# fpthink/PDGN

Measured on AMD Instinct MI355X. Metric: generator+D step points/sec (B=35, 256->2048 pts), higher is better.
Workload: dtype f32; 1 GPU; PDGNet_v2 G+D iteration (models/PDGNet_v2.py:171-256), chair-shaped synthetic batch, per-GPU batch 35, 256->2048 pts, random-init weights; global_batch=35, parallelism=dp1, losses_finite=True, hipgraph=False, issue=list

## Files before the change

include/pdgn_hip.h:

```cpp
#ifndef PDGN_HIP_H
#define PDGN_HIP_H

#include <stdint.h>

#ifdef __cplusplus
extern "C" {
#endif

#define PDGN_ERR_INVALID (-1)
#define PDGN_KNN_MAX_NSAMPLE 200

typedef void *pdgn_stream_t;

int pdgn_abi_version(void);

int pdgn_knnquery(int b, int n, int m, int nsample, const float *xyz, const float *new_xyz,
                  int32_t *idx, float *dist2, pdgn_stream_t stream);

int pdgn_grouping_forward(int b, int c, int n, int m, int nsample, const float *points,
                          const int32_t *idx, float *out, pdgn_stream_t stream);

int pdgn_grouping_backward(int b, int c, int n, int m, int nsample, const float *grad_out,
                           const int32_t *idx, float *grad_points, pdgn_stream_t stream);

// ... 54 lines not shown
                  const float *beta, const float *pre_bias, float *running_mean, float *running_var,
                  float *scratch, float *stats, pdgn_stream_t stream);
int pdgn_bn_eval_stats(int c, float eps, const float *gamma, const float *beta, const float *pre_bias,
                       const float *running_mean, const float *running_var, float *stats,
                       pdgn_stream_t stream);
int pdgn_bn_stats_from_partials(long long rows, int c, float eps, float momentum, const float *gamma,
                                const float *beta, const float *pre_bias, float *running_mean, float *running_var,
                                const float *scratch, float *stats, pdgn_stream_t stream);
int pdgn_bn_stats_from_gemm_partials(long long rows, int c, long long nparts, int block_rows, float eps, float momentum,
                                     const float *gamma, const float *beta, const float *pre_bias,
                                     float *running_mean, float *running_var, const float *partials,
                                     float *stats, double *scratch, pdgn_stream_t stream);
long long pdgn_bn_blocks_scratch_doubles(int c, long long nparts);
int pdgn_bn_act_forward(long long rows, int c, int act, const float *x, const float *stats,
                        const float *mul, float *y, int interleave_n, pdgn_stream_t stream);
int pdgn_bn_act_backward(long long rows, int c, int act, int training, const float *x,
                         const float *dy, const float *mul, const float *stats, float *scratch,
                         float *bsums, float *dx, float *dmul, int interleave_n, pdgn_stream_t stream);

long long pdgn_bn_maxpool_scratch_floats(int b, int c);
int pdgn_bn_act_maxpool(int b, int n, int c, int act, const float *x, const float *stats, float *scratch,
                        float *ymax, int32_t *yarg, pdgn_stream_t stream);
long long pdgn_bn_stats_maxpool_scratch_floats(int b, int c);
int pdgn_bn_stats_act_maxpool(int b, int n, int c, int act, float eps, float momentum, const float *x, const float *gamma,
                              const float *beta, const float *pre_bias, float *running_mean, float *running_var, float *scratch,
                              float *stats, float *ymax, int32_t *yarg, pdgn_stream_t stream);
int pdgn_bn_act_maxpool_backward(int b, int n, int c, int act, int training, const float *x,
                                 const float *dout, const int32_t *yarg, const float *stats,
                                 float *scratch, float *bsums, float *dx, pdgn_stream_t stream);
long long pdgn_dense_bn_maxpool_backward_scratch(int b, int c, int k);
int pdgn_dense_bn_maxpool_backward(int b, int n, int c, int k, int act, const float *x, const float *dout, const int32_t *yarg,
                                   const float *stats, const float *h, int ldh, const float *W, int ldw, float *scratch,
                                   float *dh, float *dW, int lddw, float *bsums, pdgn_stream_t stream);
long long pdgn_dense_bn_maxpool_input_grad_scratch(int b, int c, int k);
int pdgn_dense_bn_maxpool_input_grad(int b, int n, int c, int k, int act, const float *x, const float *dout,
                                     const int32_t *yarg, const float *stats, const float *h, int ldh,
                                     const float *W, int ldw, float *scratch, float *dh, pdgn_stream_t stream);

int pdgn_group_colsum(long long groups, long long group_rows, int c, const float *x, long long ldx, float *out,
                      pdgn_stream_t stream);

int pdgn_softmax_slots_permute(long long m, int k, int c, const float *h, float *w, pdgn_stream_t stream);
int pdgn_bn_softmax_slots_permute(long long m, int k, int c, int act, const float *x, const float *stats,
                                  float *w, pdgn_stream_t stream);
int pdgn_bn_softmax_slots_permute_mul(long long m, int k, int c, int act, const float *x, const float *stats,
                                      int act_u, const float *u, const float *stats_u, float *w, float *y,
                                      unsigned *max_out, const float *gamma_u, const float *beta_u, float bound_scale,
                                      unsigned *cmax_out, pdgn_stream_t stream);
long long pdgn_bilateral_scratch_floats(long long m, int k, int c);
int pdgn_bilateral_weighting_backward(long long m, int k, int c, int act, int training, const float *x,
                                      const float *stats_x, const float *u, const float *stats_u, const float *w,
                                      const float *dy, float *scratch, float *bsums_x, float *bsums_u, float *dx,
                                      float *du, pdgn_stream_t stream);
int pdgn_softmax_slots_permute_backward(long long m, int k, int c, const float *w, const float *dw,
                                        float *dh, pdgn_stream_t stream);

int pdgn_skinny_nt(int R, int N, int K, const float *A, int lda, const float *B, int ldb, const float *bias, float *C, int ldc,
                   pdgn_stream_t stream);
int pdgn_skinny_nn(int R, int N, int K, const float *A, int lda, const float *B, int ldb, float *C, int ldc, pdgn_stream_t stream);
int pdgn_skinny_nt_act(int R, int N, int K, const float *A, int lda, const float *B, int ldb, const float *bias, float *C, int ldc,
                       int act, pdgn_stream_t stream);
int pdgn_skinny_nn_masked(int R, int N, int K, const float *A, int lda, const float *P, int ldp, int act, const float *B,
                          int ldb, float *C, int ldc, pdgn_stream_t stream);
int pdgn_skinny_tn(int R, int N, int K, const float *A, int lda, const float *B, int ldb, float *C, int ldc, pdgn_stream_t stream);
int pdgn_split_bf16x3(int rows, int cols, const float *src, int ld_src, unsigned short *planes, int ld_planes,
                      long long plane_stride, unsigned short *planes_t, int ld_planes_t, long long plane_stride_t,
// ... 149 lines not shown
```

pdgn_amd/_lib.py:

```python
import ctypes
import os

import torch

_HERE = os.path.dirname(os.path.abspath(__file__))
SO_PATH = os.path.join(_HERE, "libpdgn_hip.so")
ABI_VERSION = 26
_lib = None


class PdgnHipError(RuntimeError):
    pass


def lib():
    global _lib
    if _lib is None:
        if not os.path.exists(SO_PATH):
            raise PdgnHipError(
                "libpdgn_hip.so is not built (%s missing): run `python -m pdgn_amd.build`; "
                "pdgn_amd has no CPU fallback" % SO_PATH)
        handle = ctypes.CDLL(SO_PATH)
        handle.pdgn_abi_version.restype = ctypes.c_int
        got = handle.pdgn_abi_version()
        if got != ABI_VERSION:
            raise PdgnHipError("libpdgn_hip.so ABI %d != expected %d: rebuild" % (got, ABI_VERSION))
        _lib = handle
        if handle.pdgn_gemm_set_mode(-1) == 2:
            ensure_scale_slots(handle=handle)
    return _lib


_SCALE_SLOTS = {}


def ensure_scale_slots(device=None, handle=None):
    if not torch.cuda.is_available():
        return
    idx = torch.cuda.current_device() if device is None or device.index is None else device.index
    if _SCALE_SLOTS.get("attached") == idx:
# ... 66 lines not shown
```

pdgn_amd/csrc/bnact.hip:

```cpp
#include "common.h"

#include "bn_geom.h"
#define ACT_NONE 0
#define ACT_RELU 1
#define ACT_LEAKY 2

__device__ __forceinline__ float act_fwd(float z, int act) {
    if (act == ACT_RELU) return fmaxf(z, 0.f);
    if (act == ACT_LEAKY) return z > 0.f ? z : 0.01f * z;
    return z;
}
__device__ __forceinline__ float act_grad(float z, int act) {
    if (act == ACT_RELU) return z > 0.f ? 1.f : 0.f;
    if (act == ACT_LEAKY) return z > 0.f ? 1.f : 0.01f;
    return 1.f;
}

struct ClGeom {
    int cg, cgb, rl;
};

__global__ __launch_bounds__(BN_THREADS) void cl_stats_kernel(long long R, int C, int cgb, int rows_per_block,
                                                              const float *__restrict__ x,
                                                              float *__restrict__ part) {
// ... 900 lines not shown
        }
    }
    const size_t blk = (size_t)b * MP_SPLIT + sp;
    float *P = part + blk * 2 * C;
    *reinterpret_cast<float4 *>(P + cgi * 4) = make_float4(s[0], s[1], s[2], s[3]);
    *reinterpret_cast<float4 *>(P + C + cgi * 4) = make_float4(q[0], q[1], q[2], q[3]);
    const size_t o = blk * C + cgi * 4;
    *reinterpret_cast<float4 *>(pmax + o) = make_float4(mx[0], mx[1], mx[2], mx[3]);
    *reinterpret_cast<int4 *>(pargmax + o) = make_int4(amx[0], amx[1], amx[2], amx[3]);
    *reinterpret_cast<float4 *>(pmin + o) = make_float4(mn[0], mn[1], mn[2], mn[3]);
    *reinterpret_cast<int4 *>(pargmin + o) = make_int4(amn[0], amn[1], amn[2], amn[3]);
}

__global__ void cl_max_pick_kernel(int B, int C, int act, const float *__restrict__ stats, const float *__restrict__ pmax,
                                   const int32_t *__restrict__ pargmax, const float *__restrict__ pmin,
                                   const int32_t *__restrict__ pargmin, float *__restrict__ ymax, int32_t *__restrict__ yarg) {
    const int e = blockIdx.x * blockDim.x + threadIdx.x;
    if (e >= B * C) return;
    const int b = e / C, c = e - b * C;
    const float sc = stats[c], sh = stats[C + c];
    const bool up = sc >= 0.f;
    const float *pv = up ? pmax : pmin;
    const int32_t *pa = up ? pargmax : pargmin;
    float best = pv[((size_t)b * MP_SPLIT) * C + c];
    int arg = pa[((size_t)b * MP_SPLIT) * C + c];
    for (int s = 1; s < MP_SPLIT; ++s) {
        const float v = pv[((size_t)b * MP_SPLIT + s) * C + c];
        if (up ? v > best : v < best) { best = v; arg = pa[((size_t)b * MP_SPLIT + s) * C + c]; }
    }
    ymax[e] = act_fwd(__fmaf_rn(best, sc, sh), act);
    yarg[e] = arg;
}

__global__ __launch_bounds__(256) void cl_max_bwd_sums_kernel(int B, int N, int C, int act, int training,
                                                              const float *__restrict__ x, const float *__restrict__ dout,
                                                              const int32_t *__restrict__ yarg, const float *__restrict__ stats,
                                                              float *__restrict__ dz, float *__restrict__ bsums,
                                                              float *__restrict__ coef, float *__restrict__ zero, int nzero) {
    __shared__ double p1[16][17], p2[16][17];
    for (int e = blockIdx.x * 256 + threadIdx.x; e < nzero; e += gridDim.x * 256) zero[e] = 0.f;
    const int cl = threadIdx.x & 15, bl = threadIdx.x >> 4;
    const int c = blockIdx.x * 16 + cl;
    double s1 = 0, s2 = 0;
    float sc = 0.f, mu = 0.f, is = 0.f;
    if (c < C) {
        sc = stats[c];
        mu = stats[2 * C + c];
        is = stats[3 * C + c];
        const float sh = stats[C + c];
        for (int b = bl; b < B; b += 16) {
            const int n = yarg[b * C + c];
            const float v = x[((size_t)b * N + n) * C + c];
            const float g = dout[b * C + c] * act_grad(__fmaf_rn(v, sc, sh), act);
            dz[b * C + c] = g;
            s1 += g;
            s2 += (double)g * (double)((v - mu) * is);
        }
    }
    p1[bl][cl] = s1;
    p2[bl][cl] = s2;
    __syncthreads();
    if (bl || c >= C) return;
    for (int q = 1; q < 16; ++q) { s1 += p1[q][cl]; s2 += p2[q][cl]; }
    bsums[c] = (float)s1;
    bsums[C + c] = (float)s2;
    float ca = 0.f, cb = 0.f;
    if (training) {
        const double R = (double)B * (double)N;
        cb = sc * is * (float)(s2 / R);
        ca = sc * (float)(s1 / R) - cb * mu;
    }
    coef[c] = ca;
    coef[C + c] = cb;
}

__global__ __launch_bounds__(BN_THREADS) void cl_max_bwd_apply_kernel(int N, int C, int cgb, const float *__restrict__ x,
                                                                      const float *__restrict__ stats,
                                                                      const float *__restrict__ coef,
                                                                      const float *__restrict__ dz,
                                                                      const int32_t *__restrict__ yarg,
                                                                      float *__restrict__ dx) {
    const int cgl = threadIdx.x % cgb, rlane = threadIdx.x / cgb, rl = BN_THREADS / cgb;
    const int cgi = blockIdx.x * cgb + cgl;
    if (cgi * 4 >= C) return;
    const int b = blockIdx.z, sp = blockIdx.y;
// ... 37 lines not shown
    hipLaunchKernelGGL(cl_apply_max_kernel, dim3(gx, MP_SPLIT, b), dim3(BN_THREADS), 0, s, n, c, cgb, act, x, stats, pmax, parg);
    hipLaunchKernelGGL(cl_max_finalize_kernel, dim3(cdiv((long long)b * c, 256)), dim3(256), 0, s, b, c, pmax, parg, ymax, yarg);
    return pdgn_launch_status();
}

extern "C" long long pdgn_bn_stats_maxpool_scratch_floats(int b, int c) { return 6LL * b * MP_SPLIT * c; }

extern "C" int pdgn_bn_stats_act_maxpool(int b, int n, int c, int act, float eps, float momentum, const float *x, const float *gamma,
                                         const float *beta, const float *pre_bias, float *running_mean, float *running_var,
                                         float *scratch, float *stats, float *ymax, int32_t *yarg, pdgn_stream_t stream) {
    if (b < 1 || n < 1 || c < 4 || c % 4 || act < 0 || act > 2 || b > 65535) return PDGN_ERR_INVALID;
    hipStream_t s = (hipStream_t)stream;
    int cgb, gx;
    mp_geometry(c, &cgb, &gx);
    const size_t bc = (size_t)b * MP_SPLIT * c;
    float *part = scratch, *pmax = part + 2 * bc, *pmin = pmax + 2 * bc;
    int32_t *pargmax = reinterpret_cast<int32_t *>(pmax + bc), *pargmin = reinterpret_cast<int32_t *>(pmin + bc);
    hipLaunchKernelGGL(cl_stats_max_kernel, dim3(gx, MP_SPLIT, b), dim3(BN_THREADS), 0, s, n, c, cgb, x, part, pmax, pargmax, pmin,
                       pargmin);
    hipLaunchKernelGGL(cl_finalize_kernel, dim3(cdiv(c, FIN_CH)), dim3(FIN_CH * FIN_PL), 0, s, (long long)b * n, c, b * MP_SPLIT, eps,
                       momentum, part, gamma, beta, pre_bias, running_mean, running_var, stats, x);
    hipLaunchKernelGGL(cl_max_pick_kernel, dim3(cdiv((long long)b * c, 256)), dim3(256), 0, s, b, c, act, stats, pmax, pargmax, pmin,
                       pargmin, ymax, yarg);
    return pdgn_launch_status();
}

extern "C" int pdgn_bn_act_maxpool_backward(int b, int n, int c, int act, int training, const float *x,
                                            const float *dout, const int32_t *yarg, const float *stats, float *scratch,
                                            float *bsums, float *dx, pdgn_stream_t stream) {
    if (b < 1 || n < 1 || c < 4 || c % 4 || act < 0 || act > 2 || b > 65535) return PDGN_ERR_INVALID;
    hipStream_t s = (hipStream_t)stream;
    float *dz = scratch, *coef = scratch + (size_t)b * c;
    hipLaunchKernelGGL(cl_max_bwd_sums_kernel, dim3(cdiv(c, 16)), dim3(256), 0, s, b, n, c, act, training, x, dout, yarg,
                       stats, dz, bsums, coef, nullptr, 0);
    int cgb, gx;
    mp_geometry(c, &cgb, &gx);
    hipLaunchKernelGGL(cl_max_bwd_apply_kernel, dim3(gx, MP_SPLIT, b), dim3(BN_THREADS), 0, s, n, c, cgb, x, stats, coef, dz,
                       yarg, dx);
    return pdgn_launch_status();
}

#define CF_TILE 32
#define CF_CSPLIT 8
#define CF_RSPLIT 32

__global__ __launch_bounds__(256) void cf_gram_kernel(int C, int K, const float *__restrict__ W, int ldw,
                                                      const float *__restrict__ coef, float *__restrict__ Gneg,
                                                      float *__restrict__ vneg) {
    __shared__ float part[3][64][20];
    const int t = threadIdx.x, o = t & 63, sl = __builtin_amdgcn_readfirstlane(t >> 6);
    const int i = blockIdx.y * CF_TILE + (o >> 3) * 4, j = blockIdx.x * CF_TILE + (o & 7) * 4;
    const bool ok = i < K && j < K, do_v = blockIdx.y == 0 && (o >> 3) == 0 && j < K;
    const int ii = min(i, K - 4), jj = min(j, K - 4);
    const int nsl = CF_CSPLIT * 4, per = (C + nsl - 1) / nsl;
    const int c0 = (blockIdx.z * 4 + sl) * per, c1 = min(C, c0 + per);
    const float *cb = coef + C;
    float acc[4][4] = {}, av[4] = {};
    for (int c = c0; c < c1; c += 8) {
        float4 wi[8], wj[8];
#pragma unroll
        for (int u = 0; u < 8; ++u) {
            const float *w = W + (size_t)min(c + u, c1 - 1) * ldw;
            wi[u] = *reinterpret_cast<const float4 *>(w + ii);
            wj[u] = *reinterpret_cast<const float4 *>(w + jj);
        }
        __builtin_amdgcn_sched_barrier(0);
#pragma unroll
// ... 152 lines not shown
                                                    float *__restrict__ dW, int lddw) {
    const int lane = threadIdx.x & 63, c = blockIdx.x * 4 + (threadIdx.x >> 6);
    if (c >= C || lane * 4 >= K) return;
    const int col = lane * 4;
    const float sc = stats[c];
    float4 acc = make_float4(0.f, 0.f, 0.f, 0.f);
    for (int b0 = 0; b0 < B; b0 += 8) {
        float4 v[8];
        float g[8];
#pragma unroll
        for (int u = 0; u < 8; ++u) {
            const int b = min(b0 + u, B - 1);
            g[u] = b0 + u < B ? sc * dz[(size_t)b * C + c] : 0.f;
            v[u] = *reinterpret_cast<const float4 *>(h + ((size_t)b * N + yarg[(size_t)b * C + c]) * ldh + col);
        }
#pragma unroll
        for (int u = 0; u < 8; ++u) {
            acc.x = __fmaf_rn(g[u], v[u].x, acc.x);
            acc.y = __fmaf_rn(g[u], v[u].y, acc.y);
            acc.z = __fmaf_rn(g[u], v[u].z, acc.z);
            acc.w = __fmaf_rn(g[u], v[u].w, acc.w);
        }
    }
    const float ca = coef[c], cb = coef[C + c];
    const float4 s = *reinterpret_cast<const float4 *>(hs + col), t = *reinterpret_cast<const float4 *>(T + (size_t)c * K + col);
    *reinterpret_cast<float4 *>(dW + (size_t)c * lddw + col) =
        make_float4(acc.x - ca * s.x - cb * t.x, acc.y - ca * s.y - cb * t.y, acc.z - ca * s.z - cb * t.z, acc.w - ca * s.w - cb * t.w);
}

extern "C" long long pdgn_dense_bn_maxpool_backward_scratch(int b, int c, int k) {
    return (long long)b * c + 2LL * c + 2LL * ((long long)k * k + k) + (long long)c * k;
}

extern "C" int pdgn_dense_bn_maxpool_backward(int b, int n, int c, int k, int act, const float *x, const float *dout,
                                              const int32_t *yarg, const float *stats, const float *h, int ldh, const float *W,
                                              int ldw, float *scratch, float *dh, float *dW, int lddw, float *bsums,
                                              pdgn_stream_t stream) {
    if (b < 1 || n < 1 || n > 65535 || c < 4 || c % 4 || k < 4 || k % 4 || k > 256 || ldw % 4 || ((uintptr_t)W & 15) ||
        ((uintptr_t)dh & 15) || act < 0 || act > 2 || b > 65535 || cf_scatter_lds(n, c) > 64 * 1024)
        return PDGN_ERR_INVALID;
    if (dW && (k < 16 || (k & (k - 1)) || ldh % 4 || lddw % 4 || ((uintptr_t)h & 15) || ((uintptr_t)dW & 15)))
        return PDGN_ERR_INVALID;
    hipStream_t s = (hipStream_t)stream;
    const size_t kk = (size_t)k * k;
    float *dz = scratch, *coef = dz + (size_t)b * c, *G = coef + 2 * (size_t)c, *v = G + kk, *H = v + k, *hs = H + kk, *T = hs + k;
    float *bs = bsums ? bsums : T;
    hipLaunchKernelGGL(cl_max_bwd_sums_kernel, dim3(cdiv(c, 16)), dim3(256), 0, s, b, n, c, act, 1, x, dout, yarg, stats, dz, bs,
                       coef, G, (int)(2 * (kk + k)));
    int rc = pdgn_launch_status();
    if (rc) return rc;
    if (dh) {
        const int gt = cdiv(k, CF_TILE);
        hipLaunchKernelGGL(cf_gram_kernel, dim3(gt, gt, CF_CSPLIT), dim3(256), 0, s, c, k, W, ldw, coef, G, v);
        if ((rc = pdgn_launch_status())) return rc;
        if ((rc = pdgn_gemm_nt((long long)b * n, k, k, h, ldh, G, k, v, nullptr, 0, dh, k, nullptr, stream))) return rc;
        hipLaunchKernelGGL(cf_scatter_kernel, dim3(CF_RSPLIT, b), dim3(256), cf_scatter_lds(n, c), s, n, c, k, W, ldw, stats, dz,
                           yarg, dh);
        if ((rc = pdgn_launch_status())) return rc;
    }
    if (dW) {
        const long long rows = (long long)b * n;
        hipLaunchKernelGGL(cf_colsum_kernel, dim3(rows >= 32768 ? 128 : (rows >= 8192 ? 64 : 16)), dim3(CFS_THREADS), 0, s, rows, k, h, ldh, hs);
        if ((rc = pdgn_launch_status())) return rc;
        if ((rc = pdgn_gemm_tn_big(rows, k, k, h, ldh, h, ldh, H, 1, stream))) return rc;
        if ((rc = pdgn_gemm_nt(c, k, k, W, ldw, H, k, nullptr, nullptr, 0, T, k, nullptr, stream))) return rc;
        hipLaunchKernelGGL(cf_dw_kernel, dim3(cdiv(c, 4)), dim3(256), 0, s, b, n, c, k, h, ldh, yarg, stats, dz, coef, hs, T, dW, lddw);
        rc = pdgn_launch_status();
    }
    return rc;
}

extern "C" long long pdgn_dense_bn_maxpool_input_grad_scratch(int b, int c, int k) {
    return pdgn_dense_bn_maxpool_backward_scratch(b, c, k);
}

extern "C" int pdgn_dense_bn_maxpool_input_grad(int b, int n, int c, int k, int act, const float *x, const float *dout,
                                                const int32_t *yarg, const float *stats, const float *h, int ldh,
                                                const float *W, int ldw, float *scratch, float *dh, pdgn_stream_t stream) {
    return pdgn_dense_bn_maxpool_backward(b, n, c, k, act, x, dout, yarg, stats, h, ldh, W, ldw, scratch, dh, nullptr, 4, nullptr,
                                          stream);
}

__global__ __launch_bounds__(256) void group_colsum_kernel(long long group_rows, int C, const float *__restrict__ x, long long ldx,
                                                           float *__restrict__ out) {
    __shared__ float4 red[256];
    const int kg = C / 4, per_pass = kg < 256 ? kg : 256;
    const int cgl = threadIdx.x % per_pass, rl = threadIdx.x / per_pass, nrl = 256 / per_pass;
    const long long g = blockIdx.y;
    const long long per = (group_rows + gridDim.x - 1) / gridDim.x, r0 = blockIdx.x * per, r1 = min(group_rows, r0 + per);
    const float *X = x + g * group_rows * ldx;
    for (int c0 = 0; c0 < kg; c0 += per_pass) {
        const int cg = c0 + cgl;
        float4 acc = make_float4(0.f, 0.f, 0.f, 0.f);
        for (long long r = r0 + rl; r < r1; r += 8 * nrl) {
            float4 v[8];
#pragma unroll
            for (int u = 0; u < 8; ++u) {
                const long long rr = r + (long long)u * nrl;
                v[u] = rr < r1 ? *reinterpret_cast<const float4 *>(X + rr * ldx + cg * 4) : make_float4(0.f, 0.f, 0.f, 0.f);
            }
#pragma unroll
            for (int u = 0; u < 8; ++u) { acc.x += v[u].x; acc.y += v[u].y; acc.z += v[u].z; acc.w += v[u].w; }
// ... 31 lines not shown
```

pdgn_amd/csrc/gemm_rp.hip:

```cpp
#include "gemm_shared.h"

typedef _Float16 rp_f16x8 __attribute__((ext_vector_type(8)));
typedef _Float16 rp_f16x2 __attribute__((ext_vector_type(2)));
typedef float rp_f32x16 __attribute__((ext_vector_type(16)));
typedef float rp_f32x2 __attribute__((ext_vector_type(2)));

struct RpArgs {
    long long M;
    int N, lda, ldw, ldc;
    const float *A;
    const unsigned short *Wp;
    long long wplane;
    float *C;
    const unsigned *max_w;
    int panels, ctiles;
    int rgroups, cslabs;
    int wg_per_xcd;
    float *stat_part;
};

__device__ __forceinline__ unsigned rp_cvt_pk(float a, float b) {
    const rp_f32x2 v = {a, b};
    return __builtin_bit_cast(unsigned, __builtin_convertvector(v, rp_f16x2));
}
// ... 300 lines not shown
}

bool rp_takes(long long m, int n, int k) {
    static const bool off = [] { const char *e = getenv("PDGN_RP"); return e && e[0] == '0'; }();
    return !off && (k == 32 || k == 64 || k == 128) && n >= 128 && m >= 4096 && (double)m * n >= 1.6e7 && m < (1LL << 28);
}

int rp_launch(long long m, int n, int k, const float *A, int lda, const unsigned short *Wp, int ldw, long long wplane, float *C, int ldc,
              float *stat_part, hipStream_t s) {
    RpArgs a;
    a.stat_part = stat_part;
    a.M = m; a.N = n; a.lda = lda; a.ldw = ldw; a.ldc = ldc; a.A = A; a.Wp = Wp; a.wplane = wplane; a.C = C;
    a.max_w = reinterpret_cast<const unsigned *>(Wp + 2 * wplane);
    a.panels = cdiv(m, 256);
    a.ctiles = cdiv(n, 64);
    static const int force_cs = [] { const char *e = getenv("PDGN_RP_CSLABS"); return e ? atoi(e) : 0; }();
    int cs = 1;
    while (cs < 8 && (double)cdiv(a.ctiles, cs) * 64 * k * 4 > 2.0e6) cs *= 2;
    if (force_cs == 1 || force_cs == 2 || force_cs == 4 || force_cs == 8) cs = force_cs;
    while (cs > 1 && (a.ctiles < cs || a.panels < 8 / cs)) cs /= 2;
    a.cslabs = cs;
    a.rgroups = 8 / cs;
    const int cus = nt_cus();
    a.wg_per_xcd = cus >= 8 ? cus / 8 : 1;
    static const int aux_env = [] { const char *e = getenv("PDGN_RP_STORE"); return e ? atoi(e) : -1; }();
    const int aux = aux_env >= 0 ? aux_env : ((double)m * n * 4 > 2.5e8 ? 2 : 0);
    static const bool pipe = [] { const char *e = getenv("PDGN_RP_PIPE"); return !(e && e[0] == '0'); }();
    const int grid = 8 * a.wg_per_xcd;
    if (k == 128) rp_go<128>(grid, s, a, aux, pipe);
    else if (k == 64) rp_go<64>(grid, s, a, aux, pipe);
    else rp_go<32>(grid, s, a, aux, pipe);
    return pdgn_launch_status();
}
```

pdgn_amd/csrc/structural.hip:

```cpp
#include "common.h"
#include <type_traits>

#define SL_THREADS 256
#define SL_TILE 2048

__global__ __launch_bounds__(SL_THREADS) void nndist_kernel(
    int n, int m, const float *__restrict__ xyz, const float *__restrict__ xyz2,
    float *__restrict__ res, int32_t *__restrict__ res_i, float *__restrict__ res2,
    int32_t *__restrict__ res2_i) {
    __shared__ float4 cand[SL_TILE];
    const int bs = blockIdx.y;
    const bool rev = blockIdx.z != 0;
    const int nq = rev ? m : n, nc = rev ? n : m;
    const float *Q = (rev ? xyz2 : xyz) + (size_t)bs * nq * 3;
    const float *C = (rev ? xyz : xyz2) + (size_t)bs * nc * 3;
    float *out = (rev ? res2 : res) + (size_t)bs * nq;
    int32_t *out_i = (rev ? res2_i : res_i) + (size_t)bs * nq;
    if ((int)(blockIdx.x * blockDim.x) >= nq) return;
    const int j = blockIdx.x * blockDim.x + threadIdx.x;
    float qx = 0.f, qy = 0.f, qz = 0.f;
    if (j < nq) { qx = Q[j * 3]; qy = Q[j * 3 + 1]; qz = Q[j * 3 + 2]; }
    float best = 0.f;
    int best_i = 0;
    for (int t0 = 0; t0 < nc; t0 += SL_TILE) {
// ... 595 lines not shown
}

extern "C" int pdgn_emd_cost_indexed(int npairs, int n, int m, const float *xyz1, const int32_t *ia,
                                     const float *xyz2, const int32_t *ib, float *temp, float *out,
                                     pdgn_stream_t stream) {
    if (!am_dims_ok(npairs, n, m)) return PDGN_ERR_INVALID;
    if (npairs == 0) return 0;
    emd_launch(npairs, n, m, xyz1, xyz2, temp, out, ia, ib, (hipStream_t)stream);
    return pdgn_launch_status();
}

extern "C" int pdgn_matchcost(int b, int n, int m, const float *xyz1, const float *xyz2,
                              const float *match, float *out, pdgn_stream_t stream) {
    if (!am_dims_ok(b, n, m)) return PDGN_ERR_INVALID;
    if (b == 0) return 0;
    hipLaunchKernelGGL(matchcost_kernel, dim3(b), dim3(AM_THREADS), 0, (hipStream_t)stream, n, m, xyz1,
                       xyz2, match, out);
    return pdgn_launch_status();
}

extern "C" int pdgn_matchcost_grad(int b, int n, int m, const float *xyz1, const float *xyz2,
                                   const float *match, float *grad1, float *grad2,
                                   pdgn_stream_t stream) {
    if (!am_dims_ok(b, n, m) || b > 65535) return PDGN_ERR_INVALID;
    if (b == 0) return 0;
    hipStream_t s = (hipStream_t)stream;
    hipLaunchKernelGGL(matchcost_grad1_kernel, dim3(cdiv(n, SL_THREADS), b), dim3(SL_THREADS), 0, s, n, m,
                       xyz1, xyz2, match, grad1);
    hipLaunchKernelGGL(matchcost_grad2_kernel, dim3(cdiv(m, SL_THREADS / PDGN_WAVE), b), dim3(SL_THREADS), 0,
                       s, n, m, xyz1, xyz2, match, grad2);
    return pdgn_launch_status();
}

extern "C" int pdgn_abi_version(void) { return 26; }
```

pdgn_amd/fused.py:

```python
import ctypes
import os
import weakref

import torch
from ._fn import Function

from . import _lib
from ._lib import check, ptr, require, stream_of

F32 = torch.float32
ACT = {"none": 0, "relu": 1, "leaky_relu": 2}


def _scratch_floats(L, rows, C):
    L.pdgn_bn_scratch_floats.restype = ctypes.c_longlong
    n = L.pdgn_bn_scratch_floats(ctypes.c_longlong(rows), C)
    if n < 0:
        raise _lib.PdgnHipError("pdgn_bn_scratch_floats: argument outside the supported range")
    return n


_ZERO_COLSUM = {}


# ... 1133 lines not shown

def _is_plain_linear_output(y2d, dense):
    fn = y2d.grad_fn
    if fn is None:
        return not y2d.requires_grad
    return (type(fn).__name__ == "LinearCLBackward" and not getattr(fn, "has_bias", True) and not getattr(fn, "has_addend", True)
            and len(fn.saved_tensors) == 2 and fn.saved_tensors[1].data_ptr() == dense.w.data_ptr()
            and fn.saved_tensors[0].data_ptr() == dense.h.data_ptr())


def _dense_input_ok(dense, x, rows, C, N):
    h, w = dense.h, dense.w
    return (x.is_cuda and h.dim() == 2 and w.dim() == 2 and h.shape[0] == rows and w.shape[0] == C and h.shape[1] == w.shape[1]
            and w.shape[1] % 4 == 0 and w.shape[1] <= 256 and w.stride(0) % 4 == 0 and w.data_ptr() % 16 == 0 and h.dtype == F32 and w.dtype == F32 and h.stride(1) == 1 and w.stride(1) == 1
            and (h.requires_grad or w.requires_grad) and rows >= _OWN_MIN_ROWS
            and (not w.requires_grad or (_CLOSED_DW and w.shape[1] >= 16 and (w.shape[1] & (w.shape[1] - 1)) == 0
                                         and h.stride(0) % 4 == 0 and h.data_ptr() % 16 == 0))
            and N <= 65535 and 2 * (N + min(N, C) + C) + 1040 + 4 * C <= 65536)


def bn_act_maxpool(x2d, bn, training, B, N, act="leaky_relu", pre_bias=None, partials=None, dense=None):
    y2d = x2d
    x2d, pre_bias = _fold_pre_bias(x2d, pre_bias, training)
    if dense is not None and not (x2d is y2d and _is_plain_linear_output(y2d, dense)):
        dense = None
    if x2d.shape[1] % 4:
        return bn_act(x2d, bn, training, act=act, pre_bias=pre_bias).view(B, N, -1).max(dim=1)[0]
    if training and bn.track_running_stats:
        _PENDING_COUNTS[bn.num_batches_tracked] = _PENDING_COUNTS.get(bn.num_batches_tracked, 0) + 1
    return BNActMaxPool.apply(x2d, bn.weight, bn.bias, bn.running_mean, bn.running_var, training, bn.momentum, bn.eps,
                              ACT[act], B, N, pre_bias, partials, dense)


class PointMax(Function):

    @staticmethod
    def forward(ctx, x):
        x = x.contiguous()
        require(x, "x", F32, 3)
        b, n, c = x.shape
        L = _lib.lib()
        L.pdgn_point_max_scratch.restype = ctypes.c_longlong
        ns = int(L.pdgn_point_max_scratch(b, n, c))
        sval = torch.empty(ns, dtype=F32, device=x.device)
        sarg = torch.empty(ns, dtype=torch.int32, device=x.device)
        out = torch.empty((b, c), dtype=F32, device=x.device)
        arg = torch.empty((b, c), dtype=torch.int32, device=x.device)
        check(L.pdgn_point_max(b, n, c, ptr(x), ptr(sval), ptr(sarg), ptr(out), ptr(arg), stream_of(x)), "pdgn_point_max")
        ctx.save_for_backward(arg)
        ctx.n = n
        return out

    @staticmethod
    def backward(ctx, g):
        arg, = ctx.saved_tensors
        b, c = arg.shape
        g = g.contiguous()
        if c % 4:
            dx = torch.zeros((b, ctx.n, c), dtype=F32, device=g.device)
            return dx.scatter_(1, arg.long().unsqueeze(1), g.unsqueeze(1))
        dx = torch.empty((b, ctx.n, c), dtype=F32, device=g.device)
        check(_lib.lib().pdgn_point_max_backward(b, ctx.n, c, ptr(g), ptr(arg), ptr(dx), stream_of(g)),
              "pdgn_point_max_backward")
        return dx


# ... 3 lines not shown
```

pdgn_amd/generator.py:

```python
import torch
import torch.nn as nn
import torch.nn.functional as F

from . import deconv as _deconv
from .deconv import PointDeconv


def _bn_act(x2d, bn, training, act="leaky_relu", pre_bias=None):
    return _deconv.bn_act(x2d, bn, training, act=act, pre_bias=pre_bias)


def _small_seq(seq, x, training):
    return _deconv.small_sequential(seq, x, training)


def _point_max(x):
    from .fused import point_max
    return point_max(x)


def _linear(rows, weight, bias=None):
    return _deconv.linear_cl(rows, weight, bias)


def _linear_stats(rows, weight, training):
    return _deconv.linear_cl(rows, weight, None, None, bool(training))


def _conv1x1_rows(rows, conv):
    return _linear(rows, _deconv._w2d(conv), conv.bias)


def _head_rows(head, x_rows, B, g=None, n_const=0):
    c0 = head[0]
    W = _deconv._w2d(c0)
    if g is not None and x_rows.is_cuda and x_rows.shape[0] >= 1024 and x_rows.shape[1] % 4 == 0 and n_const % 4 == 0:
        from .fused import HeadMLP
# ... 128 lines not shown
        for dec in self._deconvs():
            dec.drop_preassembled()


class PointDiscriminator(nn.Module):

    WIDTHS = {1: (64, 128, 256), 2: (64, 128, 256, 512), 3: (64, 128, 256, 512), 4: (64, 128, 256, 1024)}
    HIDDEN = {1: (128, 64), 2: (256, 64), 3: (256, 64), 4: (512, 256, 64)}

    def __init__(self, level, num_point=None):
        super().__init__()
        self.level = level
        self.num_point = num_point if num_point is not None else 128 << level
        layers, cin = [], 3
        for w in self.WIDTHS[level]:
            layers += [nn.Conv1d(cin, w, 1), nn.BatchNorm1d(w), nn.LeakyReLU(inplace=True)]
            cin = w
        self.fc1 = nn.Sequential(*layers)
        mlp = []
        for h in self.HIDDEN[level]:
            mlp += [nn.Linear(cin, h), nn.LeakyReLU(inplace=True)]
            cin = h
        mlp.append(nn.Linear(cin, 1))
        self.mlp = nn.Sequential(*mlp)

    def forward(self, x):
        B, _, N = x.shape
        h = x.transpose(1, 2).reshape(B * N, 3)
        last = len(self.fc1) - 3
        for i in range(0, last, 3):
            y, part = _linear_stats(h, _deconv._w2d(self.fc1[i]), self.training)
            h = _deconv.bn_act(y, self.fc1[i + 1], self.training, pre_bias=self.fc1[i].bias, partials=part)
        w_last = _deconv._w2d(self.fc1[last])
        y, part = _linear_stats(h, w_last, self.training and not _deconv.STATS_MAX)
        pooled = _deconv.bn_act_maxpool(y, self.fc1[last + 1], self.training, B, N, pre_bias=self.fc1[last].bias, partials=part,
                                        dense=_deconv.DenseInput(h, w_last))
        _deconv.flush_bn_counters()
        return _small_seq(self.mlp, pooled, self.training)


def PointDiscriminator_1(num_point=256):
    return PointDiscriminator(1, num_point)


def PointDiscriminator_2(num_point=512):
    return PointDiscriminator(2, num_point)


def PointDiscriminator_3(num_point=1024):
    return PointDiscriminator(3, num_point)


def PointDiscriminator_4(num_point=2048):
    return PointDiscriminator(4, num_point)


def load_reference_state_dict(module, state_dict):
    clean = {(k[len("module."):] if k.startswith("module.") else k): v for k, v in state_dict.items()}
    return module.load_state_dict(clean, strict=True)
```

Baseline: 3.032 million points/s.

## Fuse discriminator last-layer GEMM with BN stats and per-panel max/argmin extraction

Adds a split-f16 matrix-core GEMM kernel for the discriminator's final pointwise layer. Instead of writing the full B*N x C activation, it emits per-256-row-panel BN partial sums and column max/min with argmax/argmin. A small pick kernel then uses the sign of the BN scale to choose max or min, applies BN and the activation, and stores the picked pre-activation value. Backward reads that stored value rather than gathering from the full activation. The goal is to avoid materialising and re-reading the large final-layer output, at the cost of a new complex kernel path gated on x2 mode and shape constraints.

```diff
diff --git a/include/pdgn_hip.h b/include/pdgn_hip.h
--- a/include/pdgn_hip.h
+++ b/include/pdgn_hip.h
@@ -110,6 +110,14 @@
 int pdgn_dense_bn_maxpool_backward(int b, int n, int c, int k, int act, const float *x, const float *dout, const int32_t *yarg,
                                    const float *stats, const float *h, int ldh, const float *W, int ldw, float *scratch,
                                    float *dh, float *dW, int lddw, float *bsums, pdgn_stream_t stream);
+int pdgn_dense_bn_maxpool_backward_picked(int b, int n, int c, int k, int act, const float *ypick, const float *dout,
+                                          const int32_t *yarg, const float *stats, const float *h, int ldh, const float *W, int ldw,
+                                          float *scratch, float *dh, float *dW, int lddw, float *bsums, pdgn_stream_t stream);
+long long pdgn_dense_bn_act_maxpool_scratch_floats(int b, int n, int c);
+int pdgn_dense_bn_act_maxpool(int b, int n, int c, int k, int act, float eps, float momentum, const float *h, int ldh,
+                              const unsigned short *Wp, int ldw, long long wplane, const float *gamma, const float *beta,
+                              const float *pre_bias, float *running_mean, float *running_var, float *scratch, float *stats,
+                              float *ymax, int32_t *yarg, float *ypick, pdgn_stream_t stream);
 long long pdgn_dense_bn_maxpool_input_grad_scratch(int b, int c, int k);
 int pdgn_dense_bn_maxpool_input_grad(int b, int n, int c, int k, int act, const float *x, const float *dout,
                                      const int32_t *yarg, const float *stats, const float *h, int ldh,
diff --git a/pdgn_amd/_lib.py b/pdgn_amd/_lib.py
--- a/pdgn_amd/_lib.py
+++ b/pdgn_amd/_lib.py
@@ -5,7 +5,7 @@
 
 _HERE = os.path.dirname(os.path.abspath(__file__))
 SO_PATH = os.path.join(_HERE, "libpdgn_hip.so")
-ABI_VERSION = 26
+ABI_VERSION = 27
 _lib = None
 
 
diff --git a/pdgn_amd/csrc/bnact.hip b/pdgn_amd/csrc/bnact.hip
--- a/pdgn_amd/csrc/bnact.hip
+++ b/pdgn_amd/csrc/bnact.hip
@@ -956,11 +956,31 @@
     yarg[e] = arg;
 }
 
+__global__ void cl_ext_pick_kernel(int B, int C, int S, int act, const float *__restrict__ stats, const float *__restrict__ ext,
+                                   float *__restrict__ ymax, int32_t *__restrict__ yarg, float *__restrict__ ypick) {
+    const int e = blockIdx.x * blockDim.x + threadIdx.x;
+    if (e >= B * C) return;
+    const int b = e / C, c = e - b * C;
+    const float sc = stats[c], sh = stats[C + c];
+    const int o = sc >= 0.f ? 0 : 2 * C;
+    const float *E = ext + (size_t)b * S * 4 * C + o + c;
+    float best = E[0];
+    int arg = __float_as_int(E[C]);
+    for (int s = 1; s < S; ++s) {
+        const float v = E[(size_t)s * 4 * C];
+        if (o == 0 ? v > best : v < best) { best = v; arg = 256 * s + __float_as_int(E[(size_t)s * 4 * C + C]); }
+    }
+    ymax[e] = act_fwd(__fmaf_rn(best, sc, sh), act);
+    yarg[e] = arg;
+    ypick[e] = best;
+}
+
 __global__ __launch_bounds__(256) void cl_max_bwd_sums_kernel(int B, int N, int C, int act, int training,
                                                               const float *__restrict__ x, const float *__restrict__ dout,
                                                               const int32_t *__restrict__ yarg, const float *__restrict__ stats,
                                                               float *__restrict__ dz, float *__restrict__ bsums,
-                                                              float *__restrict__ coef, float *__restrict__ zero, int nzero) {
+                                                              float *__restrict__ coef, float *__restrict__ zero, int nzero,
+                                                              const float *__restrict__ ypick) {
     __shared__ double p1[16][17], p2[16][17];
     for (int e = blockIdx.x * 256 + threadIdx.x; e < nzero; e += gridDim.x * 256) zero[e] = 0.f;
     const int cl = threadIdx.x & 15, bl = threadIdx.x >> 4;
@@ -974,7 +994,7 @@
         const float sh = stats[C + c];
         for (int b = bl; b < B; b += 16) {
             const int n = yarg[b * C + c];
-            const float v = x[((size_t)b * N + n) * C + c];
+            const float v = ypick ? ypick[b * C + c] : x[((size_t)b * N + n) * C + c];
             const float g = dout[b * C + c] * act_grad(__fmaf_rn(v, sc, sh), act);
             dz[b * C + c] = g;
             s1 += g;
@@ -1078,7 +1098,7 @@
     hipStream_t s = (hipStream_t)stream;
     float *dz = scratch, *coef = scratch + (size_t)b * c;
     hipLaunchKernelGGL(cl_max_bwd_sums_kernel, dim3(cdiv(c, 16)), dim3(256), 0, s, b, n, c, act, training, x, dout, yarg,
-                       stats, dz, bsums, coef, nullptr, 0);
+                       stats, dz, bsums, coef, nullptr, 0, nullptr);
     int cgb, gx;
     mp_geometry(c, &cgb, &gx);
     hipLaunchKernelGGL(cl_max_bwd_apply_kernel, dim3(gx, MP_SPLIT, b), dim3(BN_THREADS), 0, s, n, c, cgb, x, stats, coef, dz,
@@ -1297,11 +1317,10 @@
     return (long long)b * c + 2LL * c + 2LL * ((long long)k * k + k) + (long long)c * k;
 }
 
-extern "C" int pdgn_dense_bn_maxpool_backward(int b, int n, int c, int k, int act, const float *x, const float *dout,
-                                              const int32_t *yarg, const float *stats, const float *h, int ldh, const float *W,
-                                              int ldw, float *scratch, float *dh, float *dW, int lddw, float *bsums,
-                                              pdgn_stream_t stream) {
-    if (b < 1 || n < 1 || n > 65535 || c < 4 || c % 4 || k < 4 || k % 4 || k > 256 || ldw % 4 || ((uintptr_t)W & 15) ||
+static int dense_bn_maxpool_backward(int b, int n, int c, int k, int act, const float *x, const float *ypick, const float *dout,
+                                     const int32_t *yarg, const float *stats, const float *h, int ldh, const float *W, int ldw,
+                                     float *scratch, float *dh, float *dW, int lddw, float *bsums, pdgn_stream_t stream) {
+    if ((!x && !ypick) || b < 1 || n < 1 || n > 65535 || c < 4 || c % 4 || k < 4 || k % 4 || k > 256 || ldw % 4 || ((uintptr_t)W & 15) ||
         ((uintptr_t)dh & 15) || act < 0 || act > 2 || b > 65535 || cf_scatter_lds(n, c) > 64 * 1024)
         return PDGN_ERR_INVALID;
     if (dW && (k < 16 || (k & (k - 1)) || ldh % 4 || lddw % 4 || ((uintptr_t)h & 15) || ((uintptr_t)dW & 15)))
@@ -1311,7 +1330,7 @@
     float *dz = scratch, *coef = dz + (size_t)b * c, *G = coef + 2 * (size_t)c, *v = G + kk, *H = v + k, *hs = H + kk, *T = hs + k;
     float *bs = bsums ? bsums : T;
     hipLaunchKernelGGL(cl_max_bwd_sums_kernel, dim3(cdiv(c, 16)), dim3(256), 0, s, b, n, c, act, 1, x, dout, yarg, stats, dz, bs,
-                       coef, G, (int)(2 * (kk + k)));
+                       coef, G, (int)(2 * (kk + k)), ypick);
     int rc = pdgn_launch_status();
     if (rc) return rc;
     if (dh) {
@@ -1333,6 +1352,54 @@
         rc = pdgn_launch_status();
     }
     return rc;
+}
+
+extern "C" int pdgn_dense_bn_maxpool_backward(int b, int n, int c, int k, int act, const float *x, const float *dout,
+                                              const int32_t *yarg, const float *stats, const float *h, int ldh, const float *W,
+                                              int ldw, float *scratch, float *dh, float *dW, int lddw, float *bsums,
+                                              pdgn_stream_t stream) {
+    return dense_bn_maxpool_backward(b, n, c, k, act, x, nullptr, dout, yarg, stats, h, ldh, W, ldw, scratch, dh, dW, lddw, bsums, stream);
+}
+
+extern "C" int pdgn_dense_bn_maxpool_backward_picked(int b, int n, int c, int k, int act, const float *ypick, const float *dout,
+                                                     const int32_t *yarg, const float *stats, const float *h, int ldh, const float *W,
+                                                     int ldw, float *scratch, float *dh, float *dW, int lddw, float *bsums,
+                                                     pdgn_stream_t stream) {
+    if (!ypick) return PDGN_ERR_INVALID;
+    return dense_bn_maxpool_backward(b, n, c, k, act, nullptr, ypick, dout, yarg, stats, h, ldh, W, ldw, scratch, dh, dW, lddw, bsums,
+                                     stream);
+}
+
+int rp_ext_launch(long long m, int n, int k, const float *A, int lda, const unsigned short *Wp, int ldw, long long wplane,
+                  float *stat_part, float *ext_part, hipStream_t s);
+
+extern "C" long long pdgn_dense_bn_act_maxpool_scratch_floats(int b, int n, int c) {
+    if (b < 1 || n < 256 || n % 256 || c < 32) return PDGN_ERR_INVALID;
+    const long long panels = (long long)b * (n / 256);
+    return 7LL * panels * c + 2 * pdgn_bn_blocks_scratch_doubles(c, panels) + 2;
+}
+
+extern "C" int pdgn_dense_bn_act_maxpool(int b, int n, int c, int k, int act, float eps, float momentum, const float *h, int ldh,
+                                         const unsigned short *Wp, int ldw, long long wplane, const float *gamma, const float *beta,
+                                         const float *pre_bias, float *running_mean, float *running_var, float *scratch, float *stats,
+                                         float *ymax, int32_t *yarg, float *ypick, pdgn_stream_t stream) {
+    if (b < 1 || b > 65535 || n < 256 || n % 256 || c < 32 || c % 32 || (k != 128 && k != 256) || act < 0 || act > 2 || ldh < k ||
+        ldh % 4 || ((uintptr_t)h & 15) || ldw < k || ldw % 8 || wplane % 8 || wplane < (long long)(c - 1) * ldw + k ||
+        ((uintptr_t)Wp & 15) || (long long)b * n * ldh >= (1LL << 31) || 2 * wplane >= (1LL << 30) || !scratch || !stats || !ymax ||
+        !yarg || !ypick)
+        return PDGN_ERR_INVALID;
+    hipStream_t s = (hipStream_t)stream;
+    const long long rows = (long long)b * n, panels = rows / 256;
+    float *part = scratch, *ext = part + 3 * panels * c;
+    double *scr = reinterpret_cast<double *>(((uintptr_t)(ext + 4 * panels * c) + 7) & ~(uintptr_t)7);
+    int rc = rp_ext_launch(rows, c, k, h, ldh, Wp, ldw, wplane, part, ext, s);
+    if (rc) return rc;
+    if ((rc = pdgn_bn_stats_from_gemm_partials(rows, c, panels, 256, eps, momentum, gamma, beta, pre_bias, running_mean, running_var,
+                                               part, stats, scr, stream)))
+        return rc;
+    hipLaunchKernelGGL(cl_ext_pick_kernel, dim3(cdiv((long long)b * c, 256)), dim3(256), 0, s, b, c, n / 256, act, stats, ext, ymax,
+                       yarg, ypick);
+    return pdgn_launch_status();
 }
 
 extern "C" long long pdgn_dense_bn_maxpool_input_grad_scratch(int b, int c, int k) {
diff --git a/pdgn_amd/csrc/gemm_rp.hip b/pdgn_amd/csrc/gemm_rp.hip
--- a/pdgn_amd/csrc/gemm_rp.hip
+++ b/pdgn_amd/csrc/gemm_rp.hip
@@ -356,3 +356,252 @@
     else rp_go<32>(grid, s, a, aux, pipe);
     return pdgn_launch_status();
 }
+
+struct RpExtArgs {
+    long long M;
+    int N, lda, ldw;
+    const float *A;
+    const unsigned short *Wp;
+    long long wplane;
+    const unsigned *max_w;
+    int panels, ctiles;
+    int rgroups, cslabs;
+    int wg_per_xcd;
+    float *stat_part, *ext_part;
+};
+
+template <int K>
+__global__ __launch_bounds__(512, 1) void gemm_rp_ext_kernel(const RpExtArgs p) {
+    static_assert(K == 128 || K == 256, "reduction lengths of the discriminators' last layers");
+    constexpr int KS = K / 16, KC = K / 32;
+    constexpr int BN = 32, BM = 256;
+    constexpr int PLANE = KC * BN * 64;
+    constexpr int WTILE = 2 * PLANE;
+    constexpr int NQ = 7;
+    constexpr int TBL = 8 * NQ * BN;
+    __shared__ __attribute__((aligned(1024))) unsigned char smem[2 * WTILE + 2 * BN * 4 + 8 * 32 * 4 + 2 * TBL * 4];
+    int *const colexp = reinterpret_cast<int *>(smem + 2 * WTILE);
+    int *const rowexp = reinterpret_cast<int *>(smem + 2 * WTILE + 2 * BN * 4);
+    float *const stl = reinterpret_cast<float *>(smem + 2 * WTILE + 2 * BN * 4 + 8 * 32 * 4);
+    const int tid = threadIdx.x, lane = tid & 63;
+    const int wave = __builtin_amdgcn_readfirstlane(tid >> 6);
+    const int li = lane & 31, lg = lane >> 5;
+
+    const int xcd = blockIdx.x & 7, slot = blockIdx.x >> 3;
+    const int rgi = xcd / p.cslabs, csi = xcd - rgi * p.cslabs;
+    const int ppg = (p.panels + p.rgroups - 1) / p.rgroups, cps = (p.ctiles + p.cslabs - 1) / p.cslabs;
+    const int p0 = rgi * ppg, p1 = min(p.panels, p0 + ppg);
+    const int c0 = csi * cps, c1 = min(p.ctiles, c0 + cps);
+    if (p0 >= p1 || c0 >= c1) return;
+    const int nc = c1 - c0;
+    const long long steps = (long long)(p1 - p0) * nc;
+    long long t = steps * slot / p.wg_per_xcd;
+    const long long t1 = steps * (slot + 1) / p.wg_per_xcd;
+    if (t >= t1) return;
+
+    constexpr int PIECES = 2 * BN * (K / 8) / 512;
+    u32x4 wraw[PIECES];
+    int craw = 0;
+    const __amdgpu_buffer_rsrc_t rsW = __builtin_amdgcn_make_buffer_rsrc((void *)p.Wp, 0, (int)min((2 * p.wplane) * 2LL, 0x7fffffffLL), 0x00020000);
+    const __amdgpu_buffer_rsrc_t rsMW = __builtin_amdgcn_make_buffer_rsrc((void *)p.max_w, 0, p.N * 4, 0x00020000);
+    auto load_w = [&](int ct) {
+        const int n0 = (c0 + ct) * BN;
+#pragma unroll
+        for (int j = 0; j < PIECES; ++j) {
+            const int id = tid + 512 * j;
+            const int part = id / (BN * (K / 8)), rem = id - part * (BN * (K / 8));
+            const int row = rem / (K / 8), c = rem - row * (K / 8);
+            const bool ok = ct < nc && n0 + row < p.N;
+            const unsigned off = (unsigned)(((long long)part * p.wplane + (long long)(n0 + row) * p.ldw + 8 * c) * 2);
+            wraw[j] = __builtin_bit_cast(u32x4, __builtin_amdgcn_raw_buffer_load_b128(rsW, ok ? off : NT_OOB, 0, 0));
+        }
+        if (tid < BN) craw = __builtin_amdgcn_raw_buffer_load_b32(rsMW, (ct < nc && n0 + tid < p.N) ? (unsigned)(n0 + tid) * 4u : NT_OOB, 0, 0);
+    };
+    auto write_w = [&](int buf) {
+#pragma unroll
+        for (int j = 0; j < PIECES; ++j) {
+            const int id = tid + 512 * j;
+            const int part = id / (BN * (K / 8)), rem = id - part * (BN * (K / 8));
+            const int row = rem / (K / 8), c = rem - row * (K / 8);
+            *reinterpret_cast<u32x4 *>(smem + buf * WTILE + part * PLANE + (c >> 2) * (BN * 64) + row * 64 + (((c & 3) ^ rp_sw(row)) * 16)) = wraw[j];
+        }
+        if (tid < BN) colexp[buf * BN + tid] = 127 - x2_scale_field((unsigned)craw);
+    };
+
+    u32x4 afh[KS], afl[KS];
+    auto load_a = [&](int panel) {
+        const long long m0 = (long long)panel * BM + 32 * wave;
+        const __amdgpu_buffer_rsrc_t rsA = __builtin_amdgcn_make_buffer_rsrc((void *)(p.A + m0 * p.lda), 0, (int)((31LL * p.lda + K) * 4), 0x00020000);
+        f32x4 raw[2 * KS];
+#pragma unroll
+        for (int s = 0; s < KS; ++s) {
+            const unsigned off = (unsigned)(li * p.lda + 16 * s + 8 * lg) * 4u;
+            raw[2 * s] = __builtin_bit_cast(f32x4, __builtin_amdgcn_raw_buffer_load_b128(rsA, off, 0, 0));
+            raw[2 * s + 1] = __builtin_bit_cast(f32x4, __builtin_amdgcn_raw_buffer_load_b128(rsA, off + 16u, 0, 0));
+        }
+        unsigned mb = 0u;
+#pragma unroll
+        for (int i = 0; i < 2 * KS; ++i)
+#pragma unroll
+            for (int r = 0; r < 4; ++r) mb = max(mb, __float_as_uint(raw[i][r]) & 0x7fffffffu);
+        mb = max(mb, (unsigned)__shfl_xor((int)mb, 32));
+        const int f = x2_scale_field(mb);
+        const float sc = __int_as_float(f << 23);
+        if (lg == 0) rowexp[wave * 32 + li] = 127 - f;
+#pragma unroll
+        for (int s = 0; s < KS; ++s)
+#pragma unroll
+            for (int e = 0; e < 4; ++e) {
+                const f32x4 v = raw[2 * s + (e >> 1)];
+                const float a2 = v[2 * (e & 1)] * sc, b2 = v[2 * (e & 1) + 1] * sc;
+                const unsigned h = rp_cvt_pk(a2, b2);
+                const rp_f16x2 hh = __builtin_bit_cast(rp_f16x2, h);
+                afh[s][e] = h;
+                afl[s][e] = rp_cvt_pk(a2 - (float)hh[0], b2 - (float)hh[1]);
+            }
+    };
+
+    auto reduce_tile = [&](const rp_f32x16 &acc, int buf, int sb) {
+        const int ec = colexp[buf * BN + li];
+        float y[16];
+#pragma unroll
+        for (int q = 0; q < 4; ++q) {
+            const i32x4 ua = *reinterpret_cast<const i32x4 *>(rowexp + wave * 32 + 8 * q + 4 * lg);
+#pragma unroll
+            for (int e = 0; e < 4; ++e) y[4 * q + e] = __builtin_ldexpf(acc[4 * q + e], ua[e] + ec);
+        }
+        const float y0 = __shfl_xor(y[0], 32);
+        const float pv = lg ? y0 : y[0];
+        float S = 0.f, Q = 0.f, mx = -INFINITY, mn = INFINITY;
+        int amx = 4 * lg, amn = 4 * lg;
+#pragma unroll
+        for (int r = 0; r < 16; ++r) {
+            const int row = (r & 3) + 8 * (r >> 2) + 4 * lg;
+            const float d = y[r] - pv;
+            S += d;
+            Q = __fmaf_rn(d, d, Q);
+            if (y[r] > mx) { mx = y[r]; amx = row; }
+            if (y[r] < mn) { mn = y[r]; amn = row; }
+        }
+        S += __shfl_xor(S, 32);
+        Q += __shfl_xor(Q, 32);
+        const float omx = __shfl_xor(mx, 32), omn = __shfl_xor(mn, 32);
+        const int oamx = __shfl_xor(amx, 32), oamn = __shfl_xor(amn, 32);
+        if (omx > mx || (omx == mx && oamx < amx)) { mx = omx; amx = oamx; }
+        if (omn < mn || (omn == mn && oamn < amn)) { mn = omn; amn = oamn; }
+        if (lg == 0) {
+            float *T = stl + sb * TBL + wave * NQ * BN + li;
+            T[0] = S;
+            T[BN] = Q;
+            T[2 * BN] = pv;
+            T[3 * BN] = mx;
+            T[4 * BN] = __int_as_float(amx);
+            T[5 * BN] = mn;
+            T[6 * BN] = __int_as_float(amn);
+        }
+    };
+    auto combine = [&](int pan, int n0, int sb) {
+        if (wave != 0 || lane >= BN) return;
+        const float *T = stl + sb * TBL + lane;
+        const float pv0 = T[2 * BN];
+        float S = T[0], Q = T[BN], mx = T[3 * BN], mn = T[5 * BN];
+        int amx = __float_as_int(T[4 * BN]), amn = __float_as_int(T[6 * BN]);
+#pragma unroll 1
+        for (int w = 1; w < 8; ++w) {
+            const float *Tw = T + w * NQ * BN;
+            const float sw = Tw[0], qw = Tw[BN], d = Tw[2 * BN] - pv0;
+            S += sw + 32.f * d;
+            Q += qw + d * (2.f * sw + 32.f * d);
+            const float vx = Tw[3 * BN], vn = Tw[5 * BN];
+            if (vx > mx) { mx = vx; amx = 32 * w + __float_as_int(Tw[4 * BN]); }
+            if (vn < mn) { mn = vn; amn = 32 * w + __float_as_int(Tw[6 * BN]); }
+        }
+        float *P = p.stat_part + (long long)pan * 3 * p.N + n0 + lane;
+        P[0] = S;
+        P[p.N] = Q;
+        P[2 * p.N] = pv0;
+        float *E = p.ext_part + (long long)pan * 4 * p.N + n0 + lane;
+        E[0] = mx;
+        E[p.N] = __int_as_float(amx);
+        E[2 * p.N] = mn;
+        E[3 * p.N] = __int_as_float(amn);
+    };
+
+    int panel = p0 + (int)(t / nc), ct = (int)(t - (long long)(panel - p0) * nc);
+    load_a(panel);
+    load_w(ct);
+    write_w(0);
+    auto next_ct = [&](int c) { return c + 1 < nc ? c + 1 : 0; };
+    load_w(t + 1 < t1 ? next_ct(ct) : nc);
+    asm volatile("s_waitcnt lgkmcnt(0)" ::: "memory");
+    __builtin_amdgcn_s_barrier();
+    asm volatile("" ::: "memory");
+
+    const unsigned w_rd = (unsigned)(li * 64 + ((lg ^ rp_sw(li)) * 16));
+    bool comb = false;
+    int comb_panel = 0, comb_n0 = 0, comb_sb = 0;
+    int buf = 0;
+    for (; t < t1; ++t) {
+        if (comb) combine(comb_panel, comb_n0, comb_sb);
+        const unsigned char *Wt = smem + buf * WTILE;
+        rp_f32x16 acc;
+#pragma unroll
+        for (int r = 0; r < 16; ++r) acc[r] = 0.f;
+        u32x4 wh[2], wl[2];
+        wh[0] = *reinterpret_cast<const u32x4 *>(Wt + w_rd);
+        wl[0] = *reinterpret_cast<const u32x4 *>(Wt + PLANE + w_rd);
+#pragma unroll
+        for (int s = 0; s < KS; ++s) {
+            if (s + 1 < KS) {
+                const unsigned o = (unsigned)(((s + 1) >> 1) * (BN * 64)) + (w_rd ^ (unsigned)(32 * ((s + 1) & 1)));
+                wh[(s + 1) & 1] = *reinterpret_cast<const u32x4 *>(Wt + o);
+                wl[(s + 1) & 1] = *reinterpret_cast<const u32x4 *>(Wt + PLANE + o);
+            }
+            acc = rp_mfma(afl[s], wh[s & 1], acc);
+            acc = rp_mfma(afh[s], wl[s & 1], acc);
+            acc = rp_mfma(afh[s], wh[s & 1], acc);
+        }
+        const int sb = (int)(t & 1);
+        reduce_tile(acc, buf, sb);
+        comb = true;
+        comb_panel = panel;
+        comb_n0 = (c0 + ct) * BN;
+        comb_sb = sb;
+        const bool more = t + 1 < t1;
+        const int nct = next_ct(ct);
+        if (more) write_w(buf ^ 1);
+        if (t + 2 < t1) load_w(next_ct(nct));
+        if (more && nct == 0) {
+            ++panel;
+            load_a(panel);
+        }
+        ct = nct;
+        buf ^= 1;
+        asm volatile("s_waitcnt lgkmcnt(0)" ::: "memory");
+        __builtin_amdgcn_s_barrier();
+        asm volatile("" ::: "memory");
+    }
+    if (comb) combine(comb_panel, comb_n0, comb_sb);
+}
+
+int rp_ext_launch(long long m, int n, int k, const float *A, int lda, const unsigned short *Wp, int ldw, long long wplane,
+                  float *stat_part, float *ext_part, hipStream_t s) {
+    RpExtArgs a;
+    a.M = m; a.N = n; a.lda = lda; a.ldw = ldw; a.A = A; a.Wp = Wp; a.wplane = wplane;
+    a.max_w = reinterpret_cast<const unsigned *>(Wp + 2 * wplane);
+    a.stat_part = stat_part;
+    a.ext_part = ext_part;
+    a.panels = (int)(m / 256);
+    a.ctiles = n / 32;
+    int cs = 1;
+    while (cs < 8 && (double)cdiv(a.ctiles, cs) * 32 * k * 4 > 2.0e6) cs *= 2;
+    while (cs > 1 && (a.ctiles < cs || a.panels < 8 / cs)) cs /= 2;
+    a.cslabs = cs;
+    a.rgroups = 8 / cs;
+    const int cus = nt_cus();
+    a.wg_per_xcd = cus >= 8 ? cus / 8 : 1;
+    const int grid = 8 * a.wg_per_xcd;
+    if (k == 256) hipLaunchKernelGGL(gemm_rp_ext_kernel<256>, dim3(grid), dim3(512), 0, s, a);
+    else hipLaunchKernelGGL(gemm_rp_ext_kernel<128>, dim3(grid), dim3(512), 0, s, a);
+    return pdgn_launch_status();
+}
diff --git a/pdgn_amd/csrc/structural.hip b/pdgn_amd/csrc/structural.hip
--- a/pdgn_amd/csrc/structural.hip
+++ b/pdgn_amd/csrc/structural.hip
@@ -651,4 +651,4 @@
     return pdgn_launch_status();
 }
 
-extern "C" int pdgn_abi_version(void) { return 26; }
+extern "C" int pdgn_abi_version(void) { return 27; }
diff --git a/pdgn_amd/fused.py b/pdgn_amd/fused.py
--- a/pdgn_amd/fused.py
+++ b/pdgn_amd/fused.py
@@ -1189,6 +1189,76 @@
                               ACT[act], B, N, pre_bias, partials, dense)
 
 
+_FUSED_DTAIL = os.environ.get("PDGN_FUSED_DTAIL", "1") == "1"
+
+
+class DenseBNActMaxPool(Function):
+
+    @staticmethod
+    def forward(ctx, h, w, bias, gamma, beta, running_mean, running_var, momentum, eps, act, B, N):
+        rows, K = h.shape
+        C = w.shape[0]
+        dev = h.device
+        L = _lib.lib()
+        _slots(w)
+        P = torch.empty(2 * C * K + 2 * C + 8, dtype=torch.int16, device=dev)
+        st = stream_of(h)
+        check(L.pdgn_split_f16x2(C, K, ptr(w), w.stride(0), ptr(P), K, ctypes.c_longlong(C * K), None, 0, ctypes.c_longlong(0), st),
+              "pdgn_split")
+        L.pdgn_dense_bn_act_maxpool_scratch_floats.restype = ctypes.c_longlong
+        scr = torch.empty(L.pdgn_dense_bn_act_maxpool_scratch_floats(B, N, C), dtype=F32, device=dev)
+        stats = torch.empty(4 * C, dtype=F32, device=dev)
+        ymax = torch.empty((B, C), dtype=F32, device=dev)
+        yarg = torch.empty((B, C), dtype=torch.int32, device=dev)
+        ypick = torch.empty((B, C), dtype=F32, device=dev)
+        pb = bias.detach().contiguous() if bias is not None else None
+        check(L.pdgn_dense_bn_act_maxpool(B, N, C, K, act, ctypes.c_float(eps), ctypes.c_float(momentum), ptr(h), h.stride(0), ptr(P), K,
+                                          ctypes.c_longlong(C * K), ptr(gamma.detach().contiguous()), ptr(beta.detach().contiguous()),
+                                          ptr(pb), ptr(running_mean), ptr(running_var), ptr(scr), ptr(stats), ptr(ymax), ptr(yarg),
+                                          ptr(ypick), st), "pdgn_dense_bn_act_maxpool")
+        ctx.save_for_backward(h, w, stats, yarg, ypick)
+        ctx.cfg = (B, N, C, K, act)
+        ctx.mark_non_differentiable(yarg)
+        return ymax
+
+    @staticmethod
+    def backward(ctx, dout):
+        h, w, stats, yarg, ypick = ctx.saved_tensors
+        B, N, C, K, act = ctx.cfg
+        dout = dout.contiguous()
+        L = _lib.lib()
+        want_h, want_w, want_bn = ctx.needs_input_grad[0], ctx.needs_input_grad[1], any(ctx.needs_input_grad[3:5])
+        L.pdgn_dense_bn_maxpool_backward_scratch.restype = ctypes.c_longlong
+        scr = torch.empty(L.pdgn_dense_bn_maxpool_backward_scratch(B, C, K), dtype=F32, device=h.device)
+        dh = torch.empty((B * N, K), dtype=F32, device=h.device) if want_h else None
+        dw = torch.empty((C, K), dtype=F32, device=h.device) if want_w else None
+        bs = torch.empty(2 * C, dtype=F32, device=h.device) if want_bn else None
+        check(L.pdgn_dense_bn_maxpool_backward_picked(B, N, C, K, act, ptr(ypick), ptr(dout), ptr(yarg), ptr(stats), ptr(h), h.stride(0),
+                                                      ptr(w), w.stride(0), ptr(scr), ptr(dh), ptr(dw), K, ptr(bs), stream_of(h)),
+              "pdgn_dense_bn_maxpool_backward_picked")
+        return (dh, dw, _pre_bias_grad(ctx.needs_input_grad[2], C, h.device), bs[C:] if want_bn else None, bs[:C] if want_bn else None,
+                None, None, None, None, None, None, None)
+
+
+def dense_tail_fusable(h, w, bias, bn, training, N):
+    if not (_FUSED_DTAIL and training and _CLOSED_TAIL and not _NO_FOLD and h.is_cuda and _lib.gemm_mode() == "x2"):
+        return False
+    if not (bn.affine and bn.track_running_stats and bn.momentum is not None and bn.running_mean is not None):
+        return False
+    if bias is not None and bias.requires_grad and not _CLOSED_DW:
+        return False
+    rows, K = h.shape if h.dim() == 2 else (0, 0)
+    C = w.shape[0]
+    return (N % 256 == 0 and K in (128, 256) and C % 32 == 0 and rows % N == 0 and h.stride(0) % 4 == 0 and h.data_ptr() % 16 == 0
+            and w.is_contiguous() and _dense_input_ok(DenseInput(h, w), h, rows, C, N))
+
+
+def dense_bn_act_maxpool(h, w, bias, bn, B, N, act="leaky_relu"):
+    if bn.track_running_stats:
+        _PENDING_COUNTS[bn.num_batches_tracked] = _PENDING_COUNTS.get(bn.num_batches_tracked, 0) + 1
+    return DenseBNActMaxPool.apply(h, w, bias, bn.weight, bn.bias, bn.running_mean, bn.running_var, bn.momentum, bn.eps, ACT[act], B, N)
+
+
 class PointMax(Function):
 
     @staticmethod
diff --git a/pdgn_amd/generator.py b/pdgn_amd/generator.py
--- a/pdgn_amd/generator.py
+++ b/pdgn_amd/generator.py
@@ -3,6 +3,7 @@
 import torch.nn.functional as F
 
 from . import deconv as _deconv
+from . import fused as _fused
 from .deconv import PointDeconv
 
 
@@ -197,6 +198,11 @@
             y, part = _linear_stats(h, _deconv._w2d(self.fc1[i]), self.training)
             h = _deconv.bn_act(y, self.fc1[i + 1], self.training, pre_bias=self.fc1[i].bias, partials=part)
         w_last = _deconv._w2d(self.fc1[last])
+        if (_deconv.linear_cl is _fused.linear_cl and _deconv.bn_act_maxpool is _fused.bn_act_maxpool
+                and _fused.dense_tail_fusable(h, w_last, self.fc1[last].bias, self.fc1[last + 1], self.training, N)):
+            pooled = _fused.dense_bn_act_maxpool(h, w_last, self.fc1[last].bias, self.fc1[last + 1], B, N)
+            _deconv.flush_bn_counters()
+            return _small_seq(self.mlp, pooled, self.training)
         y, part = _linear_stats(h, w_last, self.training and not _deconv.STATS_MAX)
         pooled = _deconv.bn_act_maxpool(y, self.fc1[last + 1], self.training, B, N, pre_bias=self.fc1[last].bias, partials=part,
                                         dense=_deconv.DenseInput(h, w_last))
```

New measurement: 3.052 million points/s (median of 6 runs). Within noise of the previous version (+0.7%).
